# facebookresearch/robust_cvd

Hardware: NVIDIA H100
Metric: flow_residual_constraints_per_sec_per_gn_iteration (higher is better)
Workload: dtype f64

## Files before the change

robust_cvd_b200/csrc/rcvd_api.cu:

```cuda
#include <algorithm>
#include <chrono>
#include <cmath>
#include <cstdarg>
#include <cstdio>
#include <cstring>
#include <dlfcn.h>
#include <limits>
#include <string>
#include <vector>

#include <cub/device/device_segmented_sort.cuh>
#include "rcvd_eval.cuh"
#include "rcvd_linalg.cuh"
#include "rcvd_update.cuh"
#include "rcvd_plan.h"
#include "rcvd_host.h"

using namespace rcvd;

static thread_local std::string g_err = "";
int set_err(int code, const char* fmt, ...) {
  char buf[512]; va_list ap; va_start(ap, fmt); vsnprintf(buf, sizeof(buf), fmt, ap); va_end(ap);
  g_err = buf; return code;
}
// ... 190 lines not shown
}
template <class T> static int upload(rcvd_problem* p, T** ptr, const std::vector<T>& v) {
  int rc = dalloc(p, ptr, v.size()); if (rc) return rc;
  if (!v.empty()) CK(cudaMemcpyAsync(*ptr, v.data(), v.size() * sizeof(T), cudaMemcpyHostToDevice, p->stream));
  return RCVD_OK;
}
static void free_all(rcvd_problem* p) {
  if (p->solve_graph) { cudaGraphExecDestroy(p->solve_graph); p->solve_graph = nullptr; }
  if (p->side_stream) cudaStreamSynchronize(p->side_stream);
  if (p->inv_stream) cudaStreamSynchronize(p->inv_stream);
  for (void* q : p->allocs) cudaFreeAsync(q, p->stream);
  p->allocs.clear();
  if (p->stream) cudaStreamSynchronize(p->stream);
  if (p->h_scal) { cudaFreeHost(p->h_scal); p->h_scal = nullptr; }
  p->structure_ready = false; p->factored = false;
}

static DevProblem dev_problem(const rcvd_problem* p) {
  DevProblem d; d.cfg = p->cfg; d.L = p->L; d.N = p->N;
  d.pairs = p->pairs.dev; d.trips = p->trips.dev; d.dpairs = p->dpairs.dev;
  d.blk_of = p->d_blk_of; d.in_range = p->d_in_range; d.median = p->d_median;
  d.adaptive = p->adaptive.empty() ? nullptr : p->d_adaptive; d.scale_locs = p->d_scale_locs;
  d.rank = p->rank; d.nranks = p->nranks;
  return d;
}

template <EvalMode MODE>
static int enqueue_residuals(rcvd_problem* p, const double* x, double* g) {
  const DevProblem d = dev_problem(p);
  const RegCounts rcn = reg_counts(p->cfg, p->L, p->N, p->nscale);
  const int regblocks = p->part_trip - p->part_reg, ntiles = p->pairs.num_tiles;
  cudaStream_t st = p->stream; double* part = p->d_partial; int rc;
  if (ntiles > 0) {
    const bool tc = MODE == EvalMode::CostGradH && p->fast_path != 0;
    if (tc && p->fast_path == 1 && p->records_sorted) rc = launch(p, k_accumulate_runs, ntiles, kTile, kRunSmem, st, false, d, x, p->d_H, g, part);
    else if (tc && fast_path_ok(p->cfg, p->L)) rc = launch(p, k_accumulate_fast, ntiles, kTile, kFastSmem, st, false, d, x, p->d_H, g, part);
    else rc = launch(p, k_pairs<MODE>, ntiles, kTile, 0, st, false, d, x, p->d_H, g, part, p->d_active);
    if (rc) return rc;
  }
  if (regblocks > 0 && (rc = launch(p, k_regularisers<MODE>, regblocks, 128, 0, st, false, d, rcn, x, p->d_H, g, part + p->part_reg, p->d_active,
                                    p->first_frame, p->last_frame))) return rc;
  if (p->trips.num_tiles > 0 && (rc = launch(p, k_triplets<MODE>, p->trips.num_tiles, kTile, 0, st, false, d, x, p->d_H, g, part + p->part_trip, p->d_active))) return rc;
  if (p->dpairs.num_tiles > 0 && (rc = launch(p, k_depth_pairs<MODE>, p->dpairs.num_tiles, kTile, 0, st, false, d, x, p->d_H, g, part + p->part_dp, p->d_active))) return rc;
  return RCVD_OK;
}

#define UP(ptr, vec) if ((rc = upload(p, &(ptr), vec))) return rc
#define DA(ptr, n) if ((rc = dalloc(p, &(ptr), (n)))) return rc
static int upload_plan(rcvd_problem* p) {
  const FactorPlan& pl = p->plan; int rc;
  UP(p->d_blk_of, pl.blk_of); UP(p->d_hblocks, pl.hblocks); UP(p->d_lblocks, pl.lblocks); UP(p->d_lvl_frames, pl.lvl_frames); UP(p->d_lvl_own, pl.lvl_own);
  UP(p->d_load_lblocks, pl.load_lblocks); UP(p->d_own_hblocks, pl.own_hblocks); UP(p->d_uperm, pl.uperm);
  UP(p->d_trsm_tasks, pl.trsm_tasks); UP(p->d_trsm_pairs, pl.trsm_pairs); UP(p->d_upd_pairs, pl.upd_pairs);
  UP(p->d_sub_tasks, pl.sub_tasks); UP(p->d_sub_need, pl.sub_need); DA(p->d_sub_counters, (size_t)4 * p->N + 4);
  UP(p->d_fwd_tasks, pl.fwd_tasks); UP(p->d_trsm_ll, pl.trsm_ll); UP(p->d_upd_items, pl.upd_items);
  return RCVD_OK;
}

static int upload_record_set(rcvd_problem* p, RecordSet& s) {
  std::vector<int32_t> frames(s.frames.size()), tile_group, tile_count; std::vector<int64_t> tile_begin;
  for (size_t i = 0; i < frames.size(); ++i) frames[i] = p->plan.iperm[s.frames[i]];
  for (int i = 0; i < s.groups(); ++i)
    for (int64_t b = s.offsets[i]; b < s.offsets[i + 1]; b += kTile) { tile_group.push_back(i); tile_begin.push_back(b); tile_count.push_back((int32_t)std::min<int64_t>(kTile, s.offsets[i + 1] - b)); }
  s.num_tiles = (int)tile_group.size();
  float* rec; int32_t *fr, *tg, *tn; int64_t* tb; int rc;
  UP(rec, s.records); UP(fr, frames); UP(tg, tile_group); UP(tb, tile_begin); UP(tn, tile_count);
  s.dev = RecordTiles{rec, fr, tg, tb, tn};
  return RCVD_OK;
}

static int set_up_problem_data(rcvd_problem* p) {
  const int N = p->N; const Layout& L = p->L; const std::vector<int>& uperm = p->plan.uperm; int rc;
  for (RecordSet* s : {&p->pairs, &p->trips, &p->dpairs}) if ((rc = upload_record_set(p, *s))) return rc;
  p->records_sorted = false;
  if (run_path_ok(p->cfg, L) && p->pairs.count() > 0 && p->pairs.count() < (int64_t)0x7fffffff) {
    const long long n = p->pairs.count();
    unsigned *d_k0 = nullptr, *d_k1 = nullptr; int *d_i0 = nullptr, *d_i1 = nullptr; float* d_sorted = nullptr; int64_t* d_off = nullptr; void* d_tmp = nullptr;
    if ((rc = dalloc(p, &d_k0, (size_t)n)) || (rc = dalloc(p, &d_k1, (size_t)n)) || (rc = dalloc(p, &d_i0, (size_t)n)) || (rc = dalloc(p, &d_i1, (size_t)n)) || (rc = dalloc(p, &d_sorted, (size_t)n * 6)) ||
        (rc = upload(p, &d_off, p->pairs.offsets))) return rc;
    if ((rc = launch(p, k_record_keys, (unsigned)((n + 255) / 256), 256, 0, p->stream, false, p->cfg, p->pairs.dev.records, n, d_k0, d_i0))) return rc;
    size_t tmp_bytes = 0;
    CK(cub::DeviceSegmentedSort::SortPairs(nullptr, tmp_bytes, d_k0, d_k1, d_i0, d_i1, (int)n, p->pairs.groups(), d_off, d_off + 1, p->stream));
    CK(cudaMallocAsync(&d_tmp, std::max<size_t>(tmp_bytes, 16), p->stream));
    CK(cub::DeviceSegmentedSort::SortPairs(d_tmp, tmp_bytes, d_k0, d_k1, d_i0, d_i1, (int)n, p->pairs.groups(), d_off, d_off + 1, p->stream));
    if ((rc = launch(p, k_gather_records, (unsigned)((n * 6 + 255) / 256), 256, 0, p->stream, false, p->pairs.dev.records, d_i1, n, d_sorted))) return rc;
    CK(cudaFreeAsync(d_tmp, p->stream));
    CK(cudaGetLastError());
    p->pairs.dev.records = d_sorted; p->records_sorted = true;
  }
  {
    std::vector<uint8_t> ir(N); std::vector<double> md(N), ad;
    for (int i = 0; i < N; ++i) { ir[i] = p->in_range[uperm[i]]; md[i] = p->median[uperm[i]]; }
    UP(p->d_in_range, ir); UP(p->d_median, md);
    if (!p->adaptive.empty()) {
      const size_t G = p->adaptive.size() / N; ad.resize(p->adaptive.size());
      for (int i = 0; i < N; ++i) std::copy(p->adaptive.begin() + (size_t)uperm[i] * G, p->adaptive.begin() + (size_t)(uperm[i] + 1) * G, ad.begin() + (size_t)i * G);
      UP(p->d_adaptive, ad);
    }
  }
  {
    std::vector<float> locs; const int gx = p->cfg.scale_grid_x, gy = p->cfg.scale_grid_y;
    for (int y = 0; y < gy; ++y) for (int x = 0; x < gx; ++x) {
      const float fx = -1.f + 2.f * x / (gx - 1);
      const float fy = -1.f + 2.f * y / (gy - 1);
      locs.push_back(fx); locs.push_back(fy);
    }
    p->nscale = (int)(locs.size() / 2);
// ... 68 lines not shown
    if (trsm_ll_smem_bytes(npad, 4) <= 220 * 1024) {
      CK(cudaFuncSetAttribute(k_trsm_ll<4>, cudaFuncAttributeMaxDynamicSharedMemorySize, (int)trsm_ll_smem_bytes(npad, 4)));
      CK(cudaFuncSetAttribute(k_trsm_ll<4, true>, cudaFuncAttributeMaxDynamicSharedMemorySize, (int)trsm_ll_smem_bytes(npad, 4)));
    }
  }
  if (potrf_smem_bytes(npad) <= 220 * 1024) CK(cudaFuncSetAttribute(k_potrf_smem, cudaFuncAttributeMaxDynamicSharedMemorySize, (int)potrf_smem_bytes(npad)));
  return RCVD_OK;
}

static int build_structure(rcvd_problem* p) {
  if (p->nranks > 1 && !p->dpairs.frames.empty()) return set_err(RCVD_ERR_INVALID, "depth-normalisation pairs are not sharded: they need a single-GPU problem (nranks = 1)");
  free_all(p);
  CK(cudaSetDevice(p->device));
  std::vector<int32_t> graph = p->struct_pairs.empty() ? p->pairs.frames : p->struct_pairs;
  graph.insert(graph.end(), p->dpairs.frames.begin(), p->dpairs.frames.end());
  if (const char* e = make_factor_plan(p->plan, p->cfg, graph, p->trips.frames, p->order_slack, p->nranks, p->rank, p->dist_enabled, p->num_sms))
    return set_err(RCVD_ERR_INVALID, "%s", e);
  while (p->ev_side.size() < 2 * p->plan.levels.size()) { cudaEvent_t e; CK(cudaEventCreateWithFlags(&e, cudaEventDisableTiming)); p->ev_side.push_back(e); }
  int rc;
  if ((rc = upload_plan(p)) || (rc = set_up_problem_data(p)) || (rc = allocate_storage(p))) return rc;
  CK(cudaStreamSynchronize(p->stream));
  p->structure_ready = true;
  return RCVD_OK;
}

static int allreduce(rcvd_problem* p, double* buf, size_t count) {
  if (p->nranks <= 1) return RCVD_OK;
  const int r = nccl::AllReduce(buf, buf, count, nccl::kFloat64, nccl::kSum, p->comm, p->stream);
  if (r != 0) return set_err(RCVD_ERR_NCCL, "ncclAllReduce failed: %s", nccl::GetErrorString ? nccl::GetErrorString(r) : "?");
  return RCVD_OK;
}
struct Seg { size_t first, count; };
static int grouped(rcvd_problem* p, double* base, size_t unit, const std::vector<Seg>& segs, bool bcast) {
  int r = nccl::GroupStart();
  for (size_t i = 0; i < segs.size() && r == 0; ++i) {
    if (segs[i].count == 0) continue;
    const int root = (int)(i % (size_t)p->nranks);
    double* ptr = base + segs[i].first * unit;
    r = bcast ? nccl::Broadcast(ptr, ptr, segs[i].count * unit, nccl::kFloat64, root, p->comm, p->stream)
              : nccl::Reduce(ptr, ptr, segs[i].count * unit, nccl::kFloat64, nccl::kSum, root, p->comm, p->stream);
  }
  const int r2 = nccl::GroupEnd();
  if (r == 0) r = r2;
  if (r != 0) return set_err(RCVD_ERR_NCCL, "grouped NCCL %s failed: %s", bcast ? "broadcast" : "reduce", nccl::GetErrorString ? nccl::GetErrorString(r) : "?");
  return RCVD_OK;
}

struct FactorSolve {
  enum { P_LOAD = 0, P_POTRF, P_TRINV, P_TRSM, P_GEMM, P_SOLVE };
  rcvd_problem* p; const FactorPlan& pl; const int N, npad, strips; cudaStream_t st, side, inv;
  int prof_level = 0;
  bool side_used = false, inv_used = false;
  int side_joined = -1;

  explicit FactorSolve(rcvd_problem* p_)
      : p(p_), pl(p_->plan), N(p_->N), npad(p_->L.npad), strips((npad + kTrsmStrip - 1) / kTrsmStrip), st(p_->stream), side(p_->side_stream),
        inv(p_->inv_stream) {}

  void mark(int cls) {
    if (!p->prof) return;
    cudaEvent_t e; cudaEventCreate(&e); cudaEventRecord(e, st); p->prof->push_back({cls < 0 ? cls : (cls | (prof_level << 8)), e});
  }
  template <class... Params, class... Args>
  int launch(int path, void (*kernel)(Params...), dim3 grid, dim3 block, size_t smem, cudaStream_t s, bool pdl, Args... args) {
    if (int rc = ::launch(p, kernel, grid, block, smem, s, pdl, args...)) return rc;
    p->paths[path]++;
    return RCVD_OK;
  }
  int wait(cudaStream_t waiter, cudaStream_t from, cudaEvent_t e) {
    CK(cudaEventRecord(e, from)); CK(cudaStreamWaitEvent(waiter, e, 0));
    return RCVD_OK;
  }
  int join_all(int level) {
    if (side_used) { if (int rc = wait(st, side, p->ev_join)) return rc; side_joined = 2 * level - 1; }
    if (inv_used) { if (int rc = wait(st, inv, p->ev_inv_join)) return rc; inv_used = false; }
    return RCVD_OK;
  }

  bool trsm_deep(const Level& v) const { return strips * v.ntrsm <= p->num_sms && trsm_ll_smem_bytes(npad, 4) <= 220 * 1024; }
  bool streamed(const Level& v) const {
    return p->use_trsm_ll && v.nown > 0 && v.ntrsm > 0 && potrf_smem_bytes(npad) <= 220 * 1024 &&
           strips * v.ntrsm <= (trsm_deep(v) ? 1 : p->trsm2_ctas_per_sm) * p->num_sms;
  }

  int factor_diagonal(const int* frames, int nfr, bool pdl) {
    if (potrf_smem_bytes(npad) <= 220 * 1024)
      return launch(LP_POTRF_SMEM, k_potrf_smem, dim3(nfr), dim3(kPotrfSmemThreads), potrf_smem_bytes(npad), st, pdl, p->d_Lb, p->d_invT, frames, npad,
                    p->d_fail, p->d_potrf_progress);
    for (int jb = 0; jb < npad / 16; ++jb) {
      if (int rc = launch(LP_POTRF_PANEL, k_potrf_panel, dim3(nfr), dim3(kPotrfThreads), 0, st, false, p->d_Lb, p->d_invT, frames, npad, jb, p->d_fail)) return rc;
      const int m = npad - (jb + 1) * 16, n64 = (m + 63) / 64;
      if (m > 0) { if (int rc = launch(LP_OTHER, k_potrf_trail, dim3(n64 * (n64 + 1) / 2, nfr), dim3(128), 0, st, false, p->d_Lb, frames, npad, jb)) return rc; }
    }
    return RCVD_OK;
  }

  int trsm(const Level& lv, const int* frames, int nfr, bool chain) {
    const bool inv_stream = p->use_trsm_ll && p->overlap;
    if (inv_stream) { if (int rc = wait(inv, st, p->ev_fork)) return rc; inv_used = true; }
    if (int rc = launch(LP_TRINV, k_trinv, dim3(npad / 16, nfr), dim3(256), (npad * 16 + 16 * (npad + 1)) * sizeof(double), inv_stream ? inv : st, false,
                        p->d_Lb, p->d_invT, p->d_invL, frames, npad)) return rc;
    mark(P_TRINV);
    if (lv.ntrsm == 0) return RCVD_OK;
    int rc;
    if (p->use_trsm_ll) {
      const bool deep = trsm_deep(lv);
// ... 5 lines not shown
      const int tiles = (npad + 63) / 64;
      rc = launch(LP_TRSM_GEMM, k_gemm_nt, dim3(tiles, tiles, lv.ntrsm), dim3(128), 0, st, false, p->d_T, p->d_Lb, p->d_invL,
                  p->d_trsm_tasks + lv.trsm_off, p->d_trsm_pairs, npad);
    }
    if (rc) return rc;
    mark(P_TRSM);
    return RCVD_OK;
  }

  int update(cudaStream_t s, int off, int n) {
    if (n <= p->num_sms)
      return launch(LP_UPD_TMA2, k_update_tma<2>, dim3(n), dim3(UpdShape<2>::threads), upd_smem_bytes(pl.upd_rb, 2), s, false,
                    p->tmapT, p->d_Lb, p->d_upd_items + off, n, p->d_upd_pairs, npad, pl.upd_neff, pl.upd_rb, 0);
    int grid = std::min(n, 2 * p->num_sms);
    if (p->upd_ipc > 0) grid = std::max(grid, (n + p->upd_ipc - 1) / p->upd_ipc);
    if (grid < n) p->paths[LP_UPD_TMA1_MULTI]++;
    return launch(LP_UPD_TMA1, k_update_tma<1>, dim3(grid), dim3(UpdShape<1>::threads), upd_smem_bytes(pl.upd_rb, 1), s, false,
                  p->tmapT, p->d_Lb, p->d_upd_items + off, n, p->d_upd_pairs, npad, pl.upd_neff, pl.upd_rb, 0);
  }

  int updates(int li) {
    const Level& lv = pl.levels[li];
    const bool u2 = lv.nit2[0] + lv.nit2[1] > 0;
    const bool fork_late = li + 1 < (int)pl.levels.size() && streamed(pl.levels[li + 1]);
    if (p->overlap && u2 && !fork_late) { if (int rc = wait(side, st, p->ev_fork)) return rc; }
    if (p->overlap) {
      int s = -1;
      for (int q = side_joined + 1; q < 2 * li; ++q) { const Level& v = pl.levels[q / 2]; if (v.nit2[q % 2] > 0 && v.join[q % 2] <= li) s = q; }
      if (s >= 0) { CK(cudaStreamWaitEvent(st, p->ev_side[s], 0)); side_joined = s; }
    }
    if (lv.nit > 0) { if (int rc = update(st, lv.it_off, lv.nit)) return rc; mark(P_GEMM); }
    if (p->overlap && u2 && fork_late) { if (int rc = wait(side, st, p->ev_fork)) return rc; }
    for (int h = 0; h < 2; ++h) if (lv.nit2[h] > 0) {
      if (int rc = update(p->overlap ? side : st, lv.it2_off[h], lv.nit2[h])) return rc;
      mark(P_GEMM);
      if (p->overlap) { CK(cudaEventRecord(p->ev_side[2 * li + h], side)); side_used = true; }
    }
    return RCVD_OK;
  }

  int broadcast_level(int li) {
    std::vector<Seg> segs;
    for (int q = 0; q < p->nranks; ++q) segs.push_back({(size_t)pl.tseg[(li * p->nranks + q) * 2], (size_t)pl.tseg[(li * p->nranks + q) * 2 + 1]});
    return grouped(p, p->d_T, (size_t)npad * npad, segs, true);
  }
  int phase_boundary() {
    if (int rc = join_all(pl.LB)) return rc;
    const size_t bsz = (size_t)npad * npad;
    std::vector<Seg> invs, tr;
    for (int q = 0; q < p->nranks; ++q) invs.push_back({(size_t)pl.fa_off[q], (size_t)pl.fa_cnt[q]});
    for (int q = 0; q < p->nranks; ++q) tr.push_back({(size_t)pl.fb_off[q], (size_t)pl.fb_cnt[q]});
    for (int q = 0; q < p->nranks; ++q) tr.push_back({(size_t)N + (size_t)pl.bseg[2 * q], (size_t)pl.bseg[2 * q + 1]});
    if (int rc = grouped(p, p->d_invL, bsz, invs, true)) return rc;
    return grouped(p, p->d_Lb, bsz, tr, true);
  }

  int substitution() {
    CK(cudaMemcpyAsync(p->d_rhs, p->d_gs, (size_t)N * npad * sizeof(double), cudaMemcpyDeviceToDevice, st));
    const int LS = pl.sub_first_level;
    int rc;
    for (int l = 0; l < LS; ++l) {
      const Level& lv = pl.levels[l];
      if ((rc = launch(LP_SUB_LEVEL, k_fwd_diag, dim3((npad + 7) / 8, lv.nframes), dim3(256), 0, st, false, p->d_invL, p->d_rhs, p->d_ytmp,
                       p->d_lvl_frames + lv.frame_off, npad))) return rc;
      if (lv.nfwd > 0 && (rc = launch(LP_SUB_LEVEL, k_fwd_update, dim3((npad + 7) / 8, lv.nfwd), dim3(256), 0, st, false, p->d_T, p->d_ytmp, p->d_rhs,
                                      p->d_fwd_tasks + lv.fwd_off, npad))) return rc;
    }
    if (LS < (int)pl.levels.size() && !pl.sub_tasks.empty()) {
      CK(cudaMemsetAsync(p->d_sub_counters, 0, ((size_t)4 * N + 4) * sizeof(int), st));
      SubCounters cn; cn.ticket = p->d_sub_counters; cn.fin = p->d_sub_counters + 4; cn.fdone = cn.fin + N; cn.bin = cn.fdone + N; cn.bdone = cn.bin + N;
      cn.fin_need = p->d_sub_need; cn.bin_need = p->d_sub_need + N;
      const int ntasks = (int)pl.sub_tasks.size();
      if ((rc = launch(LP_SUB_FUSED, k_substitution, dim3(std::min(ntasks, p->num_sms)), dim3(kSubThreads), substitution_smem_bytes(npad), st, false,
                       p->d_invL, p->d_T, p->d_rhs, p->d_ytmp, p->d_y, p->d_sub_tasks, ntasks, cn, npad))) return rc;
    }
    for (int l = LS - 1; l >= 0; --l) {
      const Level& lv = pl.levels[l];
      if (lv.nfwd > 0 && (rc = launch(LP_SUB_LEVEL, k_bwd_update, dim3((npad + 31) / 32, lv.nfwd), dim3(256), 0, st, false, p->d_T, p->d_y, p->d_ytmp,
                                      p->d_fwd_tasks + lv.fwd_off, npad))) return rc;
      if ((rc = launch(LP_SUB_LEVEL, k_bwd_diag, dim3((npad + 31) / 32, lv.nframes), dim3(256), 0, st, false, p->d_invL, p->d_ytmp, p->d_y,
                       p->d_lvl_frames + lv.frame_off, npad))) return rc;
    }
    mark(P_SOLVE);
    return RCVD_OK;
  }
};

static int enqueue_factor_solve(rcvd_problem* p) {
  FactorSolve f(p);
  const FactorPlan& pl = p->plan; const int npad = p->L.npad, nlv = (int)pl.levels.size();
  f.mark(-1);
  CK(cudaMemsetAsync(p->d_potrf_progress, 0, (size_t)p->N * sizeof(int), p->stream));
  const int nfill = (int)pl.load_lblocks.size() - pl.nload;
  if (int rc = f.launch(LP_OTHER, k_load_factor, dim3((npad * npad + 255) / 256, pl.nload + load_factor_pad_rows(npad, pl.upd_neff, nfill)), dim3(256), 0,
                        p->stream, false, p->d_H, p->d_Lb, p->d_lblocks, p->d_S, p->d_D2, npad, p->L.nf, pl.upd_neff, p->d_load_lblocks, pl.nload, nfill)) return rc;
  f.mark(FactorSolve::P_LOAD);
  for (int li = 0; li < nlv; ++li) {
    const Level& lv = pl.levels[li]; f.prof_level = li;
    if (pl.dist && li == pl.LB) { if (int rc = f.phase_boundary()) return rc; }
    if (lv.nown > 0) {
      const int* frames = p->d_lvl_own + lv.own_off;
      const bool chain = f.streamed(lv);
      if (int rc = f.factor_diagonal(frames, lv.nown, chain && li > 0)) return rc;
      f.mark(FactorSolve::P_POTRF);
      if (int rc = f.trsm(lv, frames, lv.nown, chain)) return rc;
    }
    if (pl.dist && li < pl.LB) { if (int rc = f.broadcast_level(li)) return rc; }
    if (int rc = f.updates(li)) return rc;
  }
  if (pl.dist && pl.LB >= nlv) { if (int rc = f.phase_boundary()) return rc; }
  if (int rc = f.join_all(nlv)) return rc;
  if (int rc = f.substitution()) return rc;
  CK(cudaGetLastError());
  return RCVD_OK;
}

static int factor_solve(rcvd_problem* p) {
  if (p->nranks > 1 && !p->graph_warm) {
    p->graph_warm = true; p->factored = true;
    return enqueue_factor_solve(p);
  }
  if (!p->solve_graph) {
    cudaGraph_t graph;
    const int64_t l0 = p->launches;
    int64_t paths0[LP_N]; std::copy(p->paths, p->paths + LP_N, paths0);
    CK(cudaStreamBeginCapture(p->stream, cudaStreamCaptureModeThreadLocal));
    int rc = enqueue_factor_solve(p);
    cudaError_t e = cudaStreamEndCapture(p->stream, &graph);
    for (int i = 0; i < LP_N; ++i) { p->graph_paths[i] = p->paths[i] - paths0[i]; p->paths[i] = paths0[i]; }
    if (rc) return rc;
    if (e != cudaSuccess) return set_err(RCVD_ERR_CUDA, "graph capture failed: %s", cudaGetErrorString(e));
    CK(cudaGraphInstantiate(&p->solve_graph, graph, 0));
    cudaGraphDestroy(graph);
    p->graph_launches = p->launches - l0;
    p->launches = l0;
  }
  CK(cudaGraphLaunch(p->solve_graph, p->stream));
  p->launches += p->graph_launches;
  for (int i = 0; i < LP_N; ++i) p->paths[i] += p->graph_paths[i];
  p->factored = true;
  return RCVD_OK;
}


static int enqueue_evaluate(rcvd_problem* p, const double* x, bool wantG, bool wantH, double* gout, int slot) {
  if (wantH && p->eval_only) return set_err(RCVD_ERR_INVALID, "this handle was set to evaluation-only (rcvd_debug_set_eval_only): no normal matrix");
  const Layout& L = p->L; const int N = p->N, npad = L.npad; cudaStream_t st = p->stream;
  const size_t bs = (size_t)npad * npad, Upad = (size_t)N * npad;
  if (wantH) CK(cudaMemsetAsync(p->d_H, 0, p->plan.hblocks.size() * bs * sizeof(double), st));
  if (wantG) CK(cudaMemsetAsync(gout, 0, (Upad + 8) * sizeof(double), st));
  int rc = wantH ? enqueue_residuals<EvalMode::CostGradH>(p, x, gout)
           : wantG ? enqueue_residuals<EvalMode::CostGrad>(p, x, gout) : enqueue_residuals<EvalMode::Cost>(p, x, gout);
  if (rc) return rc;
  if ((rc = launch(p, k_reduce_partials, 1, 1024, 0, st, false, p->d_partial, p->npartial, p->d_scal, slot))) return rc;
  if (p->nranks > 1) {
    if (wantG) {
      CK(cudaMemcpyAsync(gout + Upad, p->d_scal + slot, sizeof(double), cudaMemcpyDeviceToDevice, st));
      size_t cnt = Upad + 8;
      if (wantH && gout == p->d_g) { if ((rc = launch(p, k_extract_diag, (int)((Upad + 255) / 256), 256, 0, st, false, p->d_H, p->d_diagH, N, npad))) return rc; cnt = 2 * Upad + 8; }
      if ((rc = allreduce(p, gout, cnt))) return rc;
      CK(cudaMemcpyAsync(p->d_scal + slot, gout + Upad, sizeof(double), cudaMemcpyDeviceToDevice, st));
    } else if ((rc = allreduce(p, p->d_scal + slot, 1))) return rc;
    if (wantH) {
      if (p->plan.dist && !p->force_full_H) {
// ... 787 lines not shown
```

robust_cvd_b200/csrc/rcvd_linalg.cuh:

```cuda
#pragma once
#include "rcvd_device.cuh"

namespace rcvd {

constexpr int kPotrfThreads = 256;

__global__ void __launch_bounds__(kPotrfThreads) k_potrf_panel(double* __restrict__ Lb, double* __restrict__ invT,
                                                                const int* __restrict__ frames, int npad, int jb, int* __restrict__ fail) {
  __shared__ double D[16][17];
  __shared__ double Di[16][17];
  const int frame = frames[blockIdx.x];
  double* A = Lb + (size_t)frame * npad * npad;
  double* iT = invT + (size_t)frame * npad * 16;
  const int tid = threadIdx.x;
  const int j0 = jb * 16;
  {
    const int r = tid >> 4, cc = tid & 15;
    D[r][cc] = (cc <= r) ? A[(size_t)(j0 + r) * npad + j0 + cc] : 0.0;
  }
  __syncthreads();
  if (tid < 32) {
    const int i = tid;
    for (int j = 0; j < 16; ++j) {
      if (i == j) {
// ... 578 lines not shown
#pragma unroll
      for (int j = 0; j < 2; ++j) {
        double2* ptr = reinterpret_cast<double2*>(&Xs[(size_t)(wr + i * 8 + g) * ld + jt * 16 + j * 8 + 2 * t]);
        double2 v = *ptr; v.x -= acc[i][j][0]; v.y -= acc[i][j][1]; *ptr = v;
      }
    __syncwarp();
    double out[NI][2][2];
#pragma unroll
    for (int i = 0; i < NI; ++i) { out[i][0][0] = out[i][0][1] = out[i][1][0] = out[i][1][1] = 0.0; }
#pragma unroll
    for (int k4 = 0; k4 < 4; ++k4) {
      double af[NI], bf[2];
#pragma unroll
      for (int i = 0; i < NI; ++i) af[i] = Xs[(size_t)(wr + i * 8 + g) * ld + jt * 16 + k4 * 4 + t];
#pragma unroll
      for (int j = 0; j < 2; ++j) bf[j] = dsm[(j * 8 + g) * 20 + k4 * 4 + t];
#pragma unroll
      for (int i = 0; i < NI; ++i)
#pragma unroll
        for (int j = 0; j < 2; ++j) dmma_8x8x4(out[i][j][0], out[i][j][1], af[i], bf[j]);
    }
    __syncwarp();
#pragma unroll
    for (int i = 0; i < NI; ++i)
#pragma unroll
      for (int j = 0; j < 2; ++j) {
        const int r = wr + i * 8 + g, cidx = jt * 16 + j * 8 + 2 * t;
        const double2 v = make_double2(out[i][j][0], out[i][j][1]);
        *reinterpret_cast<double2*>(&Xs[(size_t)r * ld + cidx]) = v;
        if (r < rows) *reinterpret_cast<double2*>(&X[(size_t)(m0 + r) * npad + cidx]) = v;
      }
    __syncthreads();
    if constexpr (!kStreamed) stage(jt + kTrsmAhead);
  }
  if constexpr (kStreamed) asm volatile("griddepcontrol.wait;" ::: "memory");
}


__global__ void __launch_bounds__(256) k_fwd_diag(const double* __restrict__ invL, const double* __restrict__ rhs, double* __restrict__ y,
                                                   const int* __restrict__ frames, int npad) {
  const int frame = frames[blockIdx.y];
  const int row = blockIdx.x * 8 + (threadIdx.x >> 5);
  const int lane = threadIdx.x & 31;
  if (row >= npad) return;
  const double* M = invL + (size_t)frame * npad * npad + (size_t)row * npad;
  const double* b = rhs + (size_t)frame * npad;
  double s = 0.0;
  for (int q = lane; q <= row; q += 32) s += M[q] * b[q];
  s = warp_sum(s);
  if (lane == 0) y[(size_t)frame * npad + row] = s;
}
struct SolveTask { int blk; int r; int k; };
__global__ void __launch_bounds__(256) k_fwd_update(const double* __restrict__ T, const double* __restrict__ y, double* __restrict__ rhs,
                                                     const SolveTask* __restrict__ tasks, int npad) {
  const SolveTask tk = tasks[blockIdx.y];
  const int row = blockIdx.x * 8 + (threadIdx.x >> 5);
  const int lane = threadIdx.x & 31;
  if (row >= npad) return;
  const double* M = T + (size_t)tk.blk * npad * npad + (size_t)row * npad;
  const double* v = y + (size_t)tk.k * npad;
  double s = 0.0;
  for (int q = lane; q < npad; q += 32) s += M[q] * v[q];
  s = warp_sum(s);
  if (lane == 0) red_add(rhs + (size_t)tk.r * npad + row, -s);
}
__global__ void __launch_bounds__(256) k_bwd_update(const double* __restrict__ T, const double* __restrict__ x, double* __restrict__ y,
                                                     const SolveTask* __restrict__ tasks, int npad) {
  __shared__ double red[8][33];
  const SolveTask tk = tasks[blockIdx.y];
  const int cl = threadIdx.x & 31, rg = threadIdx.x >> 5;
  const int j = blockIdx.x * 32 + cl;
  double acc = 0.0;
  if (j < npad) {
    const double* M = T + (size_t)tk.blk * npad * npad + j;
    const double* xr = x + (size_t)tk.r * npad;
    for (int i = rg; i < npad; i += 8) acc += M[(size_t)i * npad] * xr[i];
  }
  red[rg][cl] = acc;
  __syncthreads();
  if (rg == 0 && j < npad) {
    double s = 0.0;
#pragma unroll
    for (int q = 0; q < 8; ++q) s += red[q][cl];
    if (s != 0.0) red_add(y + (size_t)tk.k * npad + j, -s);
  }
}
__global__ void __launch_bounds__(256) k_bwd_diag(const double* __restrict__ invL, const double* __restrict__ y, double* __restrict__ x,
                                                   const int* __restrict__ frames, int npad) {
  __shared__ double red[8][33];
  const int frame = frames[blockIdx.y];
  const int cl = threadIdx.x & 31, rg = threadIdx.x >> 5;
  const int j = blockIdx.x * 32 + cl;
  double acc = 0.0;
  if (j < npad) {
    const double* M = invL + (size_t)frame * npad * npad + j;
    const double* v = y + (size_t)frame * npad;
    const int i0 = j - (j % 8) + rg;
    for (int i = (i0 < j ? i0 + 8 : i0); i < npad; i += 8) acc += M[(size_t)i * npad] * v[i];
  }
  red[rg][cl] = acc;
  __syncthreads();
  if (rg == 0 && j < npad) {
    double s = 0.0;
#pragma unroll
    for (int q = 0; q < 8; ++q) s += red[q][cl];
    x[(size_t)frame * npad + j] = s;
  }
}

constexpr int kSubChunk = 64;
constexpr int kSubThreads = 256;
struct SubTask { int type; int blk; int r; int k; int chunk; };
struct SubCounters { int* ticket; int* fin; int* fdone; int* bin; int* bdone; const int* fin_need; const int* bin_need; };

__device__ __forceinline__ void sub_wait(const int* c, int need) { while (ld_acquire_gpu(c) < need) __nanosleep(20); }

__device__ __forceinline__ double2 ldcg2(const double* p) { return __ldcg(reinterpret_cast<const double2*>(p)); }

__global__ void __launch_bounds__(kSubThreads) k_substitution(const double* __restrict__ invL, const double* __restrict__ T, double* rhs, double* y, double* x,
                                                              const SubTask* __restrict__ tasks, int ntasks, SubCounters cn, int npad) {
  extern __shared__ __align__(16) double red[];
  __shared__ int s_task;
  const int tid = threadIdx.x, warp = tid >> 5, lane = tid & 31;
  const int nchunks = (npad + kSubChunk - 1) / kSubChunk;
  const size_t bs = (size_t)npad * npad;
  for (;;) {
    if (tid == 0) s_task = atomicAdd(cn.ticket, 1);
    __syncthreads();
    const int ti = s_task;
    if (ti >= ntasks) break;
    const SubTask tk = tasks[ti];
    const int c0 = tk.chunk * kSubChunk, c1 = min(npad, c0 + kSubChunk);
    const double* vin = tk.type == 0 ? rhs + (size_t)tk.k * npad : (tk.type == 2 ? x + (size_t)tk.r * npad : y + (size_t)tk.k * npad);
    const double* M = (tk.type == 0 || tk.type == 3) ? invL + (size_t)tk.k * bs : T + (size_t)tk.blk * bs;
    auto dep_wait = [&]() {
      if (tid == 0) {
        if (tk.type == 0) sub_wait(cn.fin + tk.k, cn.fin_need[tk.k]);
        else if (tk.type == 1) sub_wait(cn.fdone + tk.k, nchunks);
        else if (tk.type == 2) sub_wait(cn.bdone + tk.r, nchunks);
        else { sub_wait(cn.fdone + tk.k, nchunks); sub_wait(cn.bin + tk.k, cn.bin_need[tk.k]); }
      }
      __syncthreads();
    };
    if (tk.type <= 1) {
      constexpr int RW = kSubChunk / (kSubThreads / 32);
      const int r0 = c0 + warp * RW;
      double acc[RW];
#pragma unroll
      for (int i = 0; i < RW; ++i) acc[i] = 0.0;
      for (int qb = 0; qb < npad; qb += 256) {
        double2 m[4][RW];
#pragma unroll
        for (int qi = 0; qi < 4; ++qi) {
          const int q = qb + qi * 64 + 2 * lane;
#pragma unroll
          for (int i = 0; i < RW; ++i) {
            const int row = r0 + i;
            const int len = tk.type == 0 ? row + 1 : npad;
            m[qi][i] = (row < c1 && q < len) ? *reinterpret_cast<const double2*>(M + (size_t)row * npad + q) : make_double2(0.0, 0.0);
            if (q + 1 >= len) m[qi][i].y = 0.0;
          }
        }
        if (qb == 0) dep_wait();
        double2 v[4];
#pragma unroll
        for (int qi = 0; qi < 4; ++qi) { const int q = qb + qi * 64 + 2 * lane; v[qi] = q < npad ? ldcg2(vin + q) : make_double2(0.0, 0.0); }
#pragma unroll
        for (int qi = 0; qi < 4; ++qi)
#pragma unroll
          for (int i = 0; i < RW; ++i) acc[i] += m[qi][i].x * v[qi].x + m[qi][i].y * v[qi].y;
      }
#pragma unroll
      for (int i = 0; i < RW; ++i) {
        const double sum = warp_sum(acc[i]);
        const int row = r0 + i;
        if (lane == 0 && row < c1) { if (tk.type == 0) y[(size_t)tk.k * npad + row] = sum; else red_add(rhs + (size_t)tk.r * npad + row, -sum); }
      }
    } else {
      const int cl = tid & 31, rg = tid >> 5, j = c0 + 2 * cl;
      double ax = 0.0, ay = 0.0;
      const int ifirst = tk.type == 3 ? j + ((rg - j) & 7) : rg;
      for (int ib = ifirst; ib < npad || ib == ifirst; ib += 256) {
        double2 m[32];
#pragma unroll
        for (int u = 0; u < 32; ++u) { const int i = ib + 8 * u; m[u] = (i < npad && j < c1) ? *reinterpret_cast<const double2*>(M + (size_t)i * npad + j) : make_double2(0.0, 0.0); }
        if (ib == ifirst) dep_wait();
        double vi[32];
#pragma unroll
        for (int u = 0; u < 32; ++u) { const int i = ib + 8 * u; vi[u] = i < npad ? __ldcg(vin + i) : 0.0; }
#pragma unroll
        for (int u = 0; u < 32; ++u) { const int i = ib + 8 * u; ax += m[u].x * vi[u]; if (tk.type != 3 || i > j) ay += m[u].y * vi[u]; }
      }
      red[rg * (kSubChunk + 2) + 2 * cl] = ax; red[rg * (kSubChunk + 2) + 2 * cl + 1] = ay;
      __syncthreads();
      if (tid < kSubChunk && c0 + tid < c1) {
        double sum = 0.0;
#pragma unroll
        for (int q = 0; q < 8; ++q) sum += red[q * (kSubChunk + 2) + tid];
        if (tk.type == 3) x[(size_t)tk.k * npad + c0 + tid] = sum; else red_add(y + (size_t)tk.k * npad + c0 + tid, -sum);
      }
    }
    __syncthreads();
    if (tid == 0) red_release_add(tk.type == 0 ? cn.fdone + tk.k : (tk.type == 1 ? cn.fin + tk.r : (tk.type == 2 ? cn.bin + tk.k : cn.bdone + tk.k)), 1);
  }
}
__host__ __device__ inline size_t substitution_smem_bytes(int) { return (size_t)8 * (kSubChunk + 2) * sizeof(double); }

struct HBlock { int lblk; int r; int c; };
__global__ void __launch_bounds__(256) k_load_factor(const double* __restrict__ H, double* __restrict__ Lb, const HBlock* __restrict__ lb,
                                                      const double* __restrict__ S, const double* __restrict__ D2, int npad, int nf, int neff,
                                                      const int* __restrict__ blist, int nload, int nfill) {
  const size_t bs = (size_t)npad * npad;
  if ((int)blockIdx.y >= nload) {
    const int ph = npad - neff, per = ph * (npad + neff);
    const long q = ((long)(blockIdx.y - nload) * gridDim.x + blockIdx.x) * 256 + threadIdx.x;
    if (per == 0 || q >= (long)nfill * per) return;
    const int f = (int)(q / per), e = (int)(q % per), r = e - ph * npad;
    const int i = r < 0 ? neff + e / npad : r / ph, j = r < 0 ? e % npad : neff + r % ph;
    Lb[(size_t)blist[nload + f] * bs + (size_t)i * npad + j] = 0.0;
    return;
  }
  const int bid = blist[blockIdx.y];
  const HBlock b = lb[bid];
  const int e = blockIdx.x * 256 + threadIdx.x;
  if (e >= npad * npad) return;
  const int i = e / npad, j = e % npad;
  double v = 0.0;
  if (b.r == b.c) {
    if (j > i) v = 0.0;
    else if (i >= nf) v = (i == j) ? 1.0 : 0.0;
    else {
      v = H[(size_t)b.lblk * bs + e] * S[(size_t)b.r * npad + i] * S[(size_t)b.c * npad + j];
      if (i == j) v += D2[(size_t)b.r * npad + i];
    }
  } else if (i < nf && j < nf) {
    v = H[(size_t)b.lblk * bs + e] * S[(size_t)b.r * npad + i] * S[(size_t)b.c * npad + j];
  }
  Lb[(size_t)bid * bs + e] = v;
}
__host__ __device__ inline int load_factor_pad_rows(int npad, int neff, int nfill) {
  const long per = (long)(npad - neff) * (npad + neff), row = (long)((npad * npad + 255) / 256) * 256;
  return (int)(((long)nfill * per + row - 1) / row);
}

__global__ void __launch_bounds__(256) k_spmv_sym(const double* __restrict__ H, const HBlock* __restrict__ hb, const double* __restrict__ v,
                                                   double* __restrict__ out, int npad, const int* __restrict__ blist) {
  const int bid = blist ? blist[blockIdx.y] : blockIdx.y;
  const HBlock b = hb[bid];
  const int row = blockIdx.x * 8 + (threadIdx.x >> 5);
  const int lane = threadIdx.x & 31;
  if (row >= npad) return;
  const double* M = H + (size_t)bid * npad * npad + (size_t)row * npad;
  const double* vc = v + (size_t)b.c * npad;
  const double vr = v[(size_t)b.r * npad + row];
  double s = 0.0;
  if (b.r == b.c) {
// ... 18 lines not shown
```

robust_cvd_b200/csrc/rcvd_plan.h:

```cpp
#pragma once
#include <algorithm>
#include <map>
#include <set>
#include <vector>

#include "rcvd_linalg.cuh"
#include "rcvd_update.cuh"

namespace rcvd {

struct Level { int frame_off, nframes; int trsm_off, ntrsm; int upd_off, nupd; int upd2_off[2], nupd2[2]; int fwd_off, nfwd; int it_off, nit, it2_off[2], nit2[2]; int own_off, nown; int join[2]; };

constexpr int kUpdWindow = 2, kUpdWindowMaxNf = 256;

struct FactorPlan {
  std::vector<int> elim_order;
  std::vector<int> level, owner;
  std::vector<Level> levels;
  bool dist = false; int LB = 0;
  std::vector<int> uperm, iperm;
  std::vector<int> fa_off, fa_cnt, fb_off, fb_cnt, tseg, bseg, hseg;
  int nLoff = 0;
  std::vector<HBlock> hblocks, lblocks;
  std::vector<int32_t> blk_of;
// ... 178 lines not shown
    lv.trsm_off = (int)P.trsm_tasks.size(); lv.upd_off = (int)P.upd_tasks.size(); lv.fwd_off = (int)P.fwd_tasks.size();
    const bool shared_level = !dist || l >= LB;
    for (int k : lf[l]) {
      P.lvl_frames.push_back(k);
      const bool mine = shared_level || own[k] == rank;
      if (mine) P.lvl_own.push_back(k);
      for (int r : cs[k]) {
        const int id = lid[{r, k}];
        if (mine) {
          P.trsm_tasks.push_back({id - N, (int)P.trsm_pairs.size(), 1, 0});
          P.trsm_pairs.push_back(make_int2(id, k));
          P.trsm_ll.push_back({id - N, id, k});
        }
        P.fwd_tasks.push_back({id - N, r, k});
      }
    }
    lv.nown = (int)P.lvl_own.size() - lv.own_off;
    lv.join[0] = lv.join[1] = nl;
    const bool split = W > 1 && l < TB;
    for (int pass = 0; pass < 3; ++pass) {
      if (pass > 0) lv.upd2_off[pass - 1] = (int)P.upd_tasks.size();
      for (auto& tp : (pass ? deferred : late)[l]) {
        const int Lc = lvl[col_of(tp.first)];
        if (pass > 0 && (!split || Lc == l + 2) != (pass == 1)) continue;
        if (pass > 0) lv.join[pass - 1] = std::min(lv.join[pass - 1], Lc - 1);
        const bool first_fill = P.lblocks[tp.first].lblk < 0 && !updated[tp.first] && prod[tp.first][0].first == first_level[tp.first];
        updated[tp.first] = 1;
        P.upd_tasks.push_back({tp.first, (int)P.upd_pairs.size(), (int)tp.second.size(), (tp.first < N ? 1 : 0) | (first_fill ? 2 : 0)});
        { const double n = (double)L.nf; P.upd_flops += (double)tp.second.size() * (tp.first < N ? n * n * (n + 1.0) : 2.0 * n * n * n); }
        P.upd_pairs.insert(P.upd_pairs.end(), tp.second.begin(), tp.second.end());
      }
    }
    lv.ntrsm = (int)P.trsm_tasks.size() - lv.trsm_off; lv.nupd = lv.upd2_off[0] - lv.upd_off; lv.nfwd = (int)P.fwd_tasks.size() - lv.fwd_off;
    lv.nupd2[0] = lv.upd2_off[1] - lv.upd2_off[0]; lv.nupd2[1] = (int)P.upd_tasks.size() - lv.upd2_off[1];
    std::vector<UpdItem>& items = P.upd_items;
    for (int pass = 0; pass < 3; ++pass) {
      const int t0 = pass ? lv.upd2_off[pass - 1] : lv.upd_off, tn = pass ? lv.nupd2[pass - 1] : lv.nupd;
      const size_t i0 = items.size();
      for (int q = t0; q < t0 + tn; ++q) {
        const GemmTask& tk = P.upd_tasks[q];
        for (int ti = 0; ti < upd_nt; ++ti) for (int tj = 0; tj < ((tk.lower_only & 1) ? ti + 1 : upd_nt); ++tj) {
          UpdItem it; it.dst = tk.dst; it.first = tk.first; it.count = tk.count; it.m0 = (short)(ti * upd_tile); it.n0 = (short)(tj * upd_tile);
          it.mrows = (short)std::min(upd_tile, upd_neff - ti * upd_tile); it.ncols = (short)std::min(upd_tile, upd_neff - tj * upd_tile);
          it.flags = (((tk.lower_only & 1) && ti == tj) ? kUpdSymDiag : 0) | ((tk.lower_only & 2) ? kUpdFirstFill : 0);
          items.push_back(it);
        }
      }
      auto cost = [](const UpdItem& a) { return (long)a.count * (a.mrows / 8) * (a.ncols / 8) * ((a.flags & kUpdSymDiag) ? 3 : 4); };
      std::stable_sort(items.begin() + i0, items.end(), [&](const UpdItem& a, const UpdItem& b) { return cost(a) > cost(b); });
      if (pass) { lv.it2_off[pass - 1] = (int)i0; lv.nit2[pass - 1] = (int)(items.size() - i0); } else { lv.it_off = (int)i0; lv.nit = (int)(items.size() - i0); }
    }
    P.levels.push_back(lv);
  }
  P.sub_need.assign(2 * (size_t)N, 0);
  {
    const int nch = (npad + kSubChunk - 1) / kSubChunk;
    const int limit = 4 * num_sms;
    int LS = (int)P.levels.size();
    while (LS > 0 && (P.levels[LS - 1].nframes + P.levels[LS - 1].nfwd) * nch <= limit) --LS;
    P.sub_first_level = LS;
    for (size_t l = LS; l < P.levels.size(); ++l) {
      const Level& lv = P.levels[l];
      for (int i = 0; i < lv.nframes; ++i) for (int c = 0; c < nch; ++c) P.sub_tasks.push_back({0, -1, -1, P.lvl_frames[lv.frame_off + i], c});
      for (int q = 0; q < lv.nfwd; ++q) { const SolveTask& t = P.fwd_tasks[lv.fwd_off + q]; for (int c = 0; c < nch; ++c) P.sub_tasks.push_back({1, t.blk, t.r, t.k, c}); P.sub_need[t.r] += nch; P.sub_need[N + t.k] += nch; }
    }
    for (int l = (int)P.levels.size() - 1; l >= LS; --l) {
      const Level& lv = P.levels[l];
      for (int q = 0; q < lv.nfwd; ++q) { const SolveTask& t = P.fwd_tasks[lv.fwd_off + q]; for (int c = 0; c < nch; ++c) P.sub_tasks.push_back({2, t.blk, t.r, t.k, c}); }
      for (int i = 0; i < lv.nframes; ++i) for (int c = 0; c < nch; ++c) P.sub_tasks.push_back({3, -1, -1, P.lvl_frames[lv.frame_off + i], c});
    }
  }
  return nullptr;
}

}
```

Before: 85.30 million.

## Interleave forward substitution with factorization levels on a side stream

Forward substitution levels now run right after each level is factored, optionally on the inverse stream, so they overlap with the remaining factorization instead of waiting until the end. The fused persistent substitution kernel drops its forward task types and keeps only backward ones, which simplifies its dependency counters. k_fwd_update gains a rows-per-warp parameter so that fewer blocks are launched on the side stream. The risks are races between rhs/ytmp and the factor data, and extra per-level launches during factorization.

```diff
diff --git a/robust_cvd_b200/csrc/rcvd_api.cu b/robust_cvd_b200/csrc/rcvd_api.cu
--- a/robust_cvd_b200/csrc/rcvd_api.cu
+++ b/robust_cvd_b200/csrc/rcvd_api.cu
@@ -266,7 +266,7 @@
   UP(p->d_blk_of, pl.blk_of); UP(p->d_hblocks, pl.hblocks); UP(p->d_lblocks, pl.lblocks); UP(p->d_lvl_frames, pl.lvl_frames); UP(p->d_lvl_own, pl.lvl_own);
   UP(p->d_load_lblocks, pl.load_lblocks); UP(p->d_own_hblocks, pl.own_hblocks); UP(p->d_uperm, pl.uperm);
   UP(p->d_trsm_tasks, pl.trsm_tasks); UP(p->d_trsm_pairs, pl.trsm_pairs); UP(p->d_upd_pairs, pl.upd_pairs);
-  UP(p->d_sub_tasks, pl.sub_tasks); UP(p->d_sub_need, pl.sub_need); DA(p->d_sub_counters, (size_t)4 * p->N + 4);
+  UP(p->d_sub_tasks, pl.sub_tasks); UP(p->d_sub_need, pl.sub_need); DA(p->d_sub_counters, (size_t)2 * p->N + 4);
   UP(p->d_fwd_tasks, pl.fwd_tasks); UP(p->d_trsm_ll, pl.trsm_ll); UP(p->d_upd_items, pl.upd_items);
   return RCVD_OK;
 }
@@ -441,6 +441,7 @@
   int prof_level = 0;
   bool side_used = false, inv_used = false;
   int side_joined = -1;
+  int fwd_done = 0;
 
   explicit FactorSolve(rcvd_problem* p_)
       : p(p_), pl(p_->plan), N(p_->N), npad(p_->L.npad), strips((npad + kTrsmStrip - 1) / kTrsmStrip), st(p_->stream), side(p_->side_stream),
@@ -552,27 +553,38 @@
     for (int q = 0; q < p->nranks; ++q) tr.push_back({(size_t)pl.fb_off[q], (size_t)pl.fb_cnt[q]});
     for (int q = 0; q < p->nranks; ++q) tr.push_back({(size_t)N + (size_t)pl.bseg[2 * q], (size_t)pl.bseg[2 * q + 1]});
     if (int rc = grouped(p, p->d_invL, bsz, invs, true)) return rc;
-    return grouped(p, p->d_Lb, bsz, tr, true);
+    if (int rc = grouped(p, p->d_Lb, bsz, tr, true)) return rc;
+    return p->use_trsm_ll ? forward_upto(pl.LB) : RCVD_OK;
+  }
+
+  int forward(int li) {
+    const Level& lv = pl.levels[li];
+    const bool on_inv = p->use_trsm_ll && p->overlap;
+    if (on_inv) { if (int rc = wait(inv, st, p->ev_fork)) return rc; inv_used = true; }
+    cudaStream_t s = on_inv ? inv : st;
+    if (int rc = launch(LP_SUB_LEVEL, k_fwd_diag, dim3((npad + 7) / 8, lv.nframes), dim3(256), 0, s, false, p->d_invL, p->d_rhs, p->d_ytmp,
+                        p->d_lvl_frames + lv.frame_off, npad)) return rc;
+    const int rpw = on_inv ? 8 : 1;
+    if (lv.nfwd > 0) {
+      if (int rc = launch(LP_SUB_LEVEL, k_fwd_update, dim3((npad + 8 * rpw - 1) / (8 * rpw), lv.nfwd), dim3(256), 0, s, false, p->d_T, p->d_ytmp,
+                          p->d_rhs, p->d_fwd_tasks + lv.fwd_off, npad, rpw)) return rc;
+    }
+    mark(P_SOLVE);
+    return RCVD_OK;
+  }
+  int forward_upto(int end) {
+    for (; fwd_done < end; ++fwd_done) { if (int rc = forward(fwd_done)) return rc; }
+    return RCVD_OK;
   }
 
   int substitution() {
-    CK(cudaMemcpyAsync(p->d_rhs, p->d_gs, (size_t)N * npad * sizeof(double), cudaMemcpyDeviceToDevice, st));
     const int LS = pl.sub_first_level;
     int rc;
-    for (int l = 0; l < LS; ++l) {
-      const Level& lv = pl.levels[l];
-      if ((rc = launch(LP_SUB_LEVEL, k_fwd_diag, dim3((npad + 7) / 8, lv.nframes), dim3(256), 0, st, false, p->d_invL, p->d_rhs, p->d_ytmp,
-                       p->d_lvl_frames + lv.frame_off, npad))) return rc;
-      if (lv.nfwd > 0 && (rc = launch(LP_SUB_LEVEL, k_fwd_update, dim3((npad + 7) / 8, lv.nfwd), dim3(256), 0, st, false, p->d_T, p->d_ytmp, p->d_rhs,
-                                      p->d_fwd_tasks + lv.fwd_off, npad))) return rc;
-    }
     if (LS < (int)pl.levels.size() && !pl.sub_tasks.empty()) {
-      CK(cudaMemsetAsync(p->d_sub_counters, 0, ((size_t)4 * N + 4) * sizeof(int), st));
-      SubCounters cn; cn.ticket = p->d_sub_counters; cn.fin = p->d_sub_counters + 4; cn.fdone = cn.fin + N; cn.bin = cn.fdone + N; cn.bdone = cn.bin + N;
-      cn.fin_need = p->d_sub_need; cn.bin_need = p->d_sub_need + N;
+      SubCounters cn; cn.ticket = p->d_sub_counters; cn.bin = p->d_sub_counters + 4; cn.bdone = cn.bin + N; cn.bin_need = p->d_sub_need;
       const int ntasks = (int)pl.sub_tasks.size();
       if ((rc = launch(LP_SUB_FUSED, k_substitution, dim3(std::min(ntasks, p->num_sms)), dim3(kSubThreads), substitution_smem_bytes(npad), st, false,
-                       p->d_invL, p->d_T, p->d_rhs, p->d_ytmp, p->d_y, p->d_sub_tasks, ntasks, cn, npad))) return rc;
+                       p->d_invL, p->d_T, p->d_ytmp, p->d_y, p->d_sub_tasks, ntasks, cn, npad))) return rc;
     }
     for (int l = LS - 1; l >= 0; --l) {
       const Level& lv = pl.levels[l];
@@ -591,6 +603,8 @@
   const FactorPlan& pl = p->plan; const int npad = p->L.npad, nlv = (int)pl.levels.size();
   f.mark(-1);
   CK(cudaMemsetAsync(p->d_potrf_progress, 0, (size_t)p->N * sizeof(int), p->stream));
+  CK(cudaMemcpyAsync(p->d_rhs, p->d_gs, (size_t)p->N * npad * sizeof(double), cudaMemcpyDeviceToDevice, p->stream));
+  CK(cudaMemsetAsync(p->d_sub_counters, 0, ((size_t)2 * p->N + 4) * sizeof(int), p->stream));
   const int nfill = (int)pl.load_lblocks.size() - pl.nload;
   if (int rc = f.launch(LP_OTHER, k_load_factor, dim3((npad * npad + 255) / 256, pl.nload + load_factor_pad_rows(npad, pl.upd_neff, nfill)), dim3(256), 0,
                         p->stream, false, p->d_H, p->d_Lb, p->d_lblocks, p->d_S, p->d_D2, npad, p->L.nf, pl.upd_neff, p->d_load_lblocks, pl.nload, nfill)) return rc;
@@ -606,10 +620,12 @@
       if (int rc = f.trsm(lv, frames, lv.nown, chain)) return rc;
     }
     if (pl.dist && li < pl.LB) { if (int rc = f.broadcast_level(li)) return rc; }
+    if (p->use_trsm_ll && (!pl.dist || li >= pl.LB)) { if (int rc = f.forward_upto(li + 1)) return rc; }
     if (int rc = f.updates(li)) return rc;
   }
   if (pl.dist && pl.LB >= nlv) { if (int rc = f.phase_boundary()) return rc; }
   if (int rc = f.join_all(nlv)) return rc;
+  if (int rc = f.forward_upto(nlv)) return rc;
   if (int rc = f.substitution()) return rc;
   CK(cudaGetLastError());
   return RCVD_OK;
diff --git a/robust_cvd_b200/csrc/rcvd_linalg.cuh b/robust_cvd_b200/csrc/rcvd_linalg.cuh
--- a/robust_cvd_b200/csrc/rcvd_linalg.cuh
+++ b/robust_cvd_b200/csrc/rcvd_linalg.cuh
@@ -654,17 +654,18 @@
 }
 struct SolveTask { int blk; int r; int k; };
 __global__ void __launch_bounds__(256) k_fwd_update(const double* __restrict__ T, const double* __restrict__ y, double* __restrict__ rhs,
-                                                     const SolveTask* __restrict__ tasks, int npad) {
+                                                     const SolveTask* __restrict__ tasks, int npad, int rpw) {
   const SolveTask tk = tasks[blockIdx.y];
-  const int row = blockIdx.x * 8 + (threadIdx.x >> 5);
+  const int row0 = (blockIdx.x * 8 + (threadIdx.x >> 5)) * rpw;
   const int lane = threadIdx.x & 31;
-  if (row >= npad) return;
-  const double* M = T + (size_t)tk.blk * npad * npad + (size_t)row * npad;
   const double* v = y + (size_t)tk.k * npad;
-  double s = 0.0;
-  for (int q = lane; q < npad; q += 32) s += M[q] * v[q];
-  s = warp_sum(s);
-  if (lane == 0) red_add(rhs + (size_t)tk.r * npad + row, -s);
+  for (int row = row0; row < min(npad, row0 + rpw); ++row) {
+    const double* M = T + (size_t)tk.blk * npad * npad + (size_t)row * npad;
+    double s = 0.0;
+    for (int q = lane; q < npad; q += 32) s += M[q] * v[q];
+    s = warp_sum(s);
+    if (lane == 0) red_add(rhs + (size_t)tk.r * npad + row, -s);
+  }
 }
 __global__ void __launch_bounds__(256) k_bwd_update(const double* __restrict__ T, const double* __restrict__ x, double* __restrict__ y,
                                                      const SolveTask* __restrict__ tasks, int npad) {
@@ -713,17 +714,15 @@
 constexpr int kSubChunk = 64;
 constexpr int kSubThreads = 256;
 struct SubTask { int type; int blk; int r; int k; int chunk; };
-struct SubCounters { int* ticket; int* fin; int* fdone; int* bin; int* bdone; const int* fin_need; const int* bin_need; };
+struct SubCounters { int* ticket; int* bin; int* bdone; const int* bin_need; };
 
 __device__ __forceinline__ void sub_wait(const int* c, int need) { while (ld_acquire_gpu(c) < need) __nanosleep(20); }
 
-__device__ __forceinline__ double2 ldcg2(const double* p) { return __ldcg(reinterpret_cast<const double2*>(p)); }
-
-__global__ void __launch_bounds__(kSubThreads) k_substitution(const double* __restrict__ invL, const double* __restrict__ T, double* rhs, double* y, double* x,
+__global__ void __launch_bounds__(kSubThreads) k_substitution(const double* __restrict__ invL, const double* __restrict__ T, double* y, double* x,
                                                               const SubTask* __restrict__ tasks, int ntasks, SubCounters cn, int npad) {
   extern __shared__ __align__(16) double red[];
   __shared__ int s_task;
-  const int tid = threadIdx.x, warp = tid >> 5, lane = tid & 31;
+  const int tid = threadIdx.x;
   const int nchunks = (npad + kSubChunk - 1) / kSubChunk;
   const size_t bs = (size_t)npad * npad;
   for (;;) {
@@ -732,78 +731,38 @@
     const int ti = s_task;
     if (ti >= ntasks) break;
     const SubTask tk = tasks[ti];
+    const bool diag = tk.type == 1;
     const int c0 = tk.chunk * kSubChunk, c1 = min(npad, c0 + kSubChunk);
-    const double* vin = tk.type == 0 ? rhs + (size_t)tk.k * npad : (tk.type == 2 ? x + (size_t)tk.r * npad : y + (size_t)tk.k * npad);
-    const double* M = (tk.type == 0 || tk.type == 3) ? invL + (size_t)tk.k * bs : T + (size_t)tk.blk * bs;
+    const double* vin = diag ? y + (size_t)tk.k * npad : x + (size_t)tk.r * npad;
+    const double* M = diag ? invL + (size_t)tk.k * bs : T + (size_t)tk.blk * bs;
     auto dep_wait = [&]() {
-      if (tid == 0) {
-        if (tk.type == 0) sub_wait(cn.fin + tk.k, cn.fin_need[tk.k]);
-        else if (tk.type == 1) sub_wait(cn.fdone + tk.k, nchunks);
-        else if (tk.type == 2) sub_wait(cn.bdone + tk.r, nchunks);
-        else { sub_wait(cn.fdone + tk.k, nchunks); sub_wait(cn.bin + tk.k, cn.bin_need[tk.k]); }
-      }
+      if (tid == 0) { if (diag) sub_wait(cn.bin + tk.k, cn.bin_need[tk.k]); else sub_wait(cn.bdone + tk.r, nchunks); }
       __syncthreads();
     };
-    if (tk.type <= 1) {
-      constexpr int RW = kSubChunk / (kSubThreads / 32);
-      const int r0 = c0 + warp * RW;
-      double acc[RW];
-#pragma unroll
-      for (int i = 0; i < RW; ++i) acc[i] = 0.0;
-      for (int qb = 0; qb < npad; qb += 256) {
-        double2 m[4][RW];
-#pragma unroll
-        for (int qi = 0; qi < 4; ++qi) {
-          const int q = qb + qi * 64 + 2 * lane;
-#pragma unroll
-          for (int i = 0; i < RW; ++i) {
-            const int row = r0 + i;
-            const int len = tk.type == 0 ? row + 1 : npad;
-            m[qi][i] = (row < c1 && q < len) ? *reinterpret_cast<const double2*>(M + (size_t)row * npad + q) : make_double2(0.0, 0.0);
-            if (q + 1 >= len) m[qi][i].y = 0.0;
-          }
-        }
-        if (qb == 0) dep_wait();
-        double2 v[4];
-#pragma unroll
-        for (int qi = 0; qi < 4; ++qi) { const int q = qb + qi * 64 + 2 * lane; v[qi] = q < npad ? ldcg2(vin + q) : make_double2(0.0, 0.0); }
-#pragma unroll
-        for (int qi = 0; qi < 4; ++qi)
-#pragma unroll
-          for (int i = 0; i < RW; ++i) acc[i] += m[qi][i].x * v[qi].x + m[qi][i].y * v[qi].y;
-      }
-#pragma unroll
-      for (int i = 0; i < RW; ++i) {
-        const double sum = warp_sum(acc[i]);
-        const int row = r0 + i;
-        if (lane == 0 && row < c1) { if (tk.type == 0) y[(size_t)tk.k * npad + row] = sum; else red_add(rhs + (size_t)tk.r * npad + row, -sum); }
-      }
-    } else {
-      const int cl = tid & 31, rg = tid >> 5, j = c0 + 2 * cl;
-      double ax = 0.0, ay = 0.0;
-      const int ifirst = tk.type == 3 ? j + ((rg - j) & 7) : rg;
-      for (int ib = ifirst; ib < npad || ib == ifirst; ib += 256) {
-        double2 m[32];
-#pragma unroll
-        for (int u = 0; u < 32; ++u) { const int i = ib + 8 * u; m[u] = (i < npad && j < c1) ? *reinterpret_cast<const double2*>(M + (size_t)i * npad + j) : make_double2(0.0, 0.0); }
-        if (ib == ifirst) dep_wait();
-        double vi[32];
-#pragma unroll
-        for (int u = 0; u < 32; ++u) { const int i = ib + 8 * u; vi[u] = i < npad ? __ldcg(vin + i) : 0.0; }
-#pragma unroll
-        for (int u = 0; u < 32; ++u) { const int i = ib + 8 * u; ax += m[u].x * vi[u]; if (tk.type != 3 || i > j) ay += m[u].y * vi[u]; }
-      }
-      red[rg * (kSubChunk + 2) + 2 * cl] = ax; red[rg * (kSubChunk + 2) + 2 * cl + 1] = ay;
-      __syncthreads();
-      if (tid < kSubChunk && c0 + tid < c1) {
-        double sum = 0.0;
-#pragma unroll
-        for (int q = 0; q < 8; ++q) sum += red[q * (kSubChunk + 2) + tid];
-        if (tk.type == 3) x[(size_t)tk.k * npad + c0 + tid] = sum; else red_add(y + (size_t)tk.k * npad + c0 + tid, -sum);
-      }
-    }
-    __syncthreads();
-    if (tid == 0) red_release_add(tk.type == 0 ? cn.fdone + tk.k : (tk.type == 1 ? cn.fin + tk.r : (tk.type == 2 ? cn.bin + tk.k : cn.bdone + tk.k)), 1);
+    const int cl = tid & 31, rg = tid >> 5, j = c0 + 2 * cl;
+    double ax = 0.0, ay = 0.0;
+    const int ifirst = diag ? j + ((rg - j) & 7) : rg;
+    for (int ib = ifirst; ib < npad || ib == ifirst; ib += 256) {
+      double2 m[32];
+#pragma unroll
+      for (int u = 0; u < 32; ++u) { const int i = ib + 8 * u; m[u] = (i < npad && j < c1) ? *reinterpret_cast<const double2*>(M + (size_t)i * npad + j) : make_double2(0.0, 0.0); }
+      if (ib == ifirst) dep_wait();
+      double vi[32];
+#pragma unroll
+      for (int u = 0; u < 32; ++u) { const int i = ib + 8 * u; vi[u] = i < npad ? __ldcg(vin + i) : 0.0; }
+#pragma unroll
+      for (int u = 0; u < 32; ++u) { const int i = ib + 8 * u; ax += m[u].x * vi[u]; if (!diag || i > j) ay += m[u].y * vi[u]; }
+    }
+    red[rg * (kSubChunk + 2) + 2 * cl] = ax; red[rg * (kSubChunk + 2) + 2 * cl + 1] = ay;
+    __syncthreads();
+    if (tid < kSubChunk && c0 + tid < c1) {
+      double sum = 0.0;
+#pragma unroll
+      for (int q = 0; q < 8; ++q) sum += red[q * (kSubChunk + 2) + tid];
+      if (diag) x[(size_t)tk.k * npad + c0 + tid] = sum; else red_add(y + (size_t)tk.k * npad + c0 + tid, -sum);
+    }
+    __syncthreads();
+    if (tid == 0) red_release_add(diag ? cn.bdone + tk.k : cn.bin + tk.k, 1);
   }
 }
 __host__ __device__ inline size_t substitution_smem_bytes(int) { return (size_t)8 * (kSubChunk + 2) * sizeof(double); }
diff --git a/robust_cvd_b200/csrc/rcvd_plan.h b/robust_cvd_b200/csrc/rcvd_plan.h
--- a/robust_cvd_b200/csrc/rcvd_plan.h
+++ b/robust_cvd_b200/csrc/rcvd_plan.h
@@ -254,22 +254,17 @@
     }
     P.levels.push_back(lv);
   }
-  P.sub_need.assign(2 * (size_t)N, 0);
+  P.sub_need.assign((size_t)N, 0);
   {
     const int nch = (npad + kSubChunk - 1) / kSubChunk;
     const int limit = 4 * num_sms;
     int LS = (int)P.levels.size();
     while (LS > 0 && (P.levels[LS - 1].nframes + P.levels[LS - 1].nfwd) * nch <= limit) --LS;
     P.sub_first_level = LS;
-    for (size_t l = LS; l < P.levels.size(); ++l) {
-      const Level& lv = P.levels[l];
-      for (int i = 0; i < lv.nframes; ++i) for (int c = 0; c < nch; ++c) P.sub_tasks.push_back({0, -1, -1, P.lvl_frames[lv.frame_off + i], c});
-      for (int q = 0; q < lv.nfwd; ++q) { const SolveTask& t = P.fwd_tasks[lv.fwd_off + q]; for (int c = 0; c < nch; ++c) P.sub_tasks.push_back({1, t.blk, t.r, t.k, c}); P.sub_need[t.r] += nch; P.sub_need[N + t.k] += nch; }
-    }
     for (int l = (int)P.levels.size() - 1; l >= LS; --l) {
       const Level& lv = P.levels[l];
-      for (int q = 0; q < lv.nfwd; ++q) { const SolveTask& t = P.fwd_tasks[lv.fwd_off + q]; for (int c = 0; c < nch; ++c) P.sub_tasks.push_back({2, t.blk, t.r, t.k, c}); }
-      for (int i = 0; i < lv.nframes; ++i) for (int c = 0; c < nch; ++c) P.sub_tasks.push_back({3, -1, -1, P.lvl_frames[lv.frame_off + i], c});
+      for (int q = 0; q < lv.nfwd; ++q) { const SolveTask& t = P.fwd_tasks[lv.fwd_off + q]; for (int c = 0; c < nch; ++c) P.sub_tasks.push_back({0, t.blk, t.r, t.k, c}); P.sub_need[t.k] += nch; }
+      for (int i = 0; i < lv.nframes; ++i) for (int c = 0; c < nch; ++c) P.sub_tasks.push_back({1, -1, -1, P.lvl_frames[lv.frame_off + i], c});
     }
   }
   return nullptr;
```

After: 87.13 million (median of 6 runs). 1.02x the previous value.
